# Lainshower/debiasing-multi-modal

Measured on AMD Instinct MI355X. Metric: images/sec (embed+adapter step), CLIP-RN50 224px bs=1024, higher is better.
Workload: dtype f32; 1 GPU; CLIP-RN50 224px encode_image + adapter(1024-128-1024) CE/SGD step, 1024 images/GPU, global batch 1024 (the metric's configuration, CLIP-RN50 224px bs=1024 on one GPU); global_batch=1024, batch_per_gpu=1024, parallelism=dp1, collective=none

## Files before the change

### debiasing-multi-modal_amd/_lib.py

```python
import ctypes
import glob
import os
import subprocess
from ctypes import c_double, c_float, c_int, c_int64, c_size_t, c_void_p

_HERE = os.path.dirname(os.path.abspath(__file__))
CSRC = os.path.join(_HERE, "csrc")
LIB_PATH = os.environ.get("DBMM_LIB") or os.path.join(_HERE, "libdbmm_hip.so")
INCLUDE = os.path.join(os.path.dirname(_HERE), "include")

_lib = None


def sources():
    return sorted(glob.glob(os.path.join(CSRC, "*.hip")))


KERNEL_SOURCES = (
    ("igemm_", ("igemm_f32.hip", "igemm_epilogue.inc", "common.h")),
    ("bottleneck_chain_kernel", ("bottleneck_chain.hip", "common.h")),
    ("bottleneck_chain8_kernel", ("bottleneck_chain8.hip", "common.h")),
    ("conv3x3_c32_kernel", ("conv_patch.hip", "common.h")),
    ("gemm_pair_8ph_kernel", ("gemm_pair_8ph.hip", "gemm_pair_8ph_epilogue.inc", "persistent_tiles.h", "common.h")),
    ("conv3x3_halo8", ("conv3x3_halo8.hip", "conv3x3_halo8_epilogue.inc", "persistent_tiles.h", "common.h")),
# ... 67 lines not shown

_SIGS = {
    "dbmm_set_option": [ctypes.c_char_p, _I],
    "dbmm_get_option": [ctypes.c_char_p, ctypes.POINTER(ctypes.c_int)],
    "dbmm_version": [],
    "dbmm_error_string": [_I],
    "dbmm_conv_bn_act": [_P, _P, _P, _P, _P, _L, _L, _L, _L, _L, _L, _L, _L, _L, _I, _P],
    "dbmm_conv1x1_bn_act": [_P, _P, _P, _P, _P, _L, _L, _L, _L, _L, _I, _P],
    "dbmm_conv3x3_bn_act": [_P, _P, _P, _P, _P, _L, _L, _L, _L, _L, _I, _P],
    "dbmm_gemm_bias_act": [_P, _L, _I, _P, _L, _I, _P, _P, _L, _P, _L, _L, _L, _L, _F, _I, _P],
    "dbmm_workspace_bytes_igemm": [],
    "dbmm_debug_last_igemm": [_P],
    "dbmm_conv_bn_act_ws": [_P, _P, _P, _P, _P, _L, _L, _L, _L, _L, _L, _L, _L, _L, _I, _I, _P, _Z, _P],
    "dbmm_gemm_bias_act_ws": [_P, _L, _I, _P, _L, _I, _P, _P, _L, _P, _L, _L, _L, _L, _F, _I, _P, _Z, _P],
    "dbmm_split_planes_bytes": [_L, _L],
    "dbmm_split_weight_planes": [_P, _P, _L, _L, _P],
    "dbmm_conv_bn_act_x3": [_P, _P, _P, _P, _P, _P, _L, _L, _L, _L, _L, _L, _L, _L, _L, _I, _I, _P, _Z, _P],
    "dbmm_split_planes_f16_bytes": [_L, _L],
    "dbmm_split_weight_planes_f16": [_P, _P, _L, _L, _I, _P],
    "dbmm_conv_bn_act_x2": [_P, _P, _P, _P, _I, _I, _P, _P, _P, _P, _P, _P, _L, _L, _L, _L, _L, _L, _L, _L, _L, _I, _I, _I, _P, _Z, _P],
    "dbmm_gemm_bias_act_x2": [_P, _L, _P, _P, _P, _I, _I, _L, _P, _P, _P, _L, _P, _L, _P, _L, _L, _L, _F, _I, _P, _Z, _P],
    "dbmm_gemm_dual_bn_act_x2": [_P, _L, _P, _P, _I, _L, _L, _P, _P, _L, _P, _P, _L, _L, _P, _P, _P, _L, _P, _L, _L, _I, _P, _Z, _P],
    "dbmm_bottleneck_chain_x2": [_P, _P, _P, _I, _P, _P, _P, _P, _P, _P, _P, _I, _P, _P, _P, _P, _L, _L, _L, _L, _L, _L, _P],
    "dbmm_bottleneck_chain_dual_x2": [_P, _P, _P, _I, _P, _P, _P, _P, _P, _P, _P, _P, _P, _I, _P, _P, _P, _P, _L, _L, _L, _L, _L, _P],
    "dbmm_gemm_f16": [_P, _L, _P, _L, _P, _P, _L, _P, _L, _L, _L, _L, _I, _P],
    "dbmm_gemm_f16_ws": [_P, _L, _P, _L, _P, _P, _L, _P, _L, _L, _L, _L, _I, _P, _Z, _P],
    "dbmm_mha_core_f16": [_P, _P, _L, _L, _L, _L, _I, _P],
    "dbmm_layernorm_f16": [_P, _L, _P, _P, _P, _L, _L, _L, _F, _P],
    "dbmm_conv1x1_bn_act_f16": [_P, _P, _P, _P, _P, _P, _L, _L, _L, _I, _P],
    "dbmm_conv1x1_bn_act_f16_ws": [_P, _P, _P, _P, _P, _P, _L, _L, _L, _I, _P, _Z, _P],
    "dbmm_conv1x1_dual_bn_act_f16": [_P, _P, _P, _P, _P, _P, _P, _P, _L, _L, _L, _L, _I, _P],
    "dbmm_bottleneck_chain_f16": [_P, _P, _P, _P, _P, _P, _P, _P, _P, _P, _L, _L, _L, _L, _P],
    "dbmm_bottleneck_chain_pool_f16": [_P, _P, _P, _P, _P, _P, _P, _P, _P, _P, _P, _L, _L, _L, _L, _L, _L, _P],
    "dbmm_bottleneck_chain_dual_f16": [_P, _P, _P, _P, _P, _P, _P, _P, _P, _P, _P, _P, _L, _L, _L, _L, _L, _P],
    "dbmm_conv3x3_bn_relu_f16": [_P, _P, _P, _P, _P, _L, _L, _L, _L, _L, _I, _P],
    "dbmm_conv_stem_s2_f16": [_P, _I, _P, _P, _P, _L, _L, _L, _L, _P],
    "dbmm_conv1x1_res_pool_f16": [_P, _P, _P, _P, _P, _P, _P, _L, _L, _L, _L, _L, _P],
    "dbmm_conv_stem_s2_bn_f16": [_P, _I, _P, _P, _P, _P, _L, _L, _L, _L, _P],
    "dbmm_avgpool2_f16": [_P, _P, _L, _L, _L, _L, _P],
    "dbmm_im2col_patch_f16": [_P, _I, _P, _L, _L, _L, _L, _P],
    "dbmm_vit_tokens_f16": [_P, _P, _P, _P, _L, _L, _L, _P],
    "dbmm_embed_gather_f16": [_P, _P, _P, _P, _L, _L, _L, _L, _P],
    "dbmm_gather_eot_f16": [_P, _P, _P, _L, _L, _L, _P],
    "dbmm_cast_f32_f16": [_P, _P, _L, _P],
    "dbmm_conv3x3_c32_bn_relu_x2": [_P, _P, _P, _I, _P, _P, _P, _P, _L, _L, _L, _L, _L, _I, _P],
    "dbmm_bottleneck_block_chain_x2": [_P, _P, _P, _I, _P, _P, _P, _I, _P, _P, _P, _P, _P, _P, _P, _P, _P, _P, _I, _P, _P, _P, _P,
                                       _L, _L, _L, _L, _L, _L, _P],
    "dbmm_gemm_bias_act_x3": [_P, _L, _P, _P, _L, _P, _P, _L, _P, _L, _L, _L, _L, _F, _I, _P, _Z, _P],
    "dbmm_gemm_batched": [_P, _L, _L, _I, _P, _L, _L, _I, _P, _L, _P, _L, _L, _L, _L, _L, _L, _F, _I, _P],
    "dbmm_gemm_pair_8ph": [_P, _L, _P, _P, _I, _L, _P, _P, _P, _L, _P, _L, _P, _L, _L, _L, _F, _I, _P],
    "dbmm_conv_stem_s2": [_P, _P, _P, _P, _P, _L, _L, _L, _L, _P],
    "dbmm_avgpool2d": [_P, _P, _L, _L, _L, _L, _L, _P],
    "dbmm_workspace_bytes_attnpool": [_L, _L, _L],
    "dbmm_attnpool": [_P, _P, _P, _P, _P, _P, _P, _P, _P, _L, _L, _L, _L, _L, _P, _Z, _P],
    "dbmm_attnpool_x": [_P, _I, _P, _P, _P, _P, _P, _P, _P, _P, _L, _L, _L, _L, _L, _P, _Z, _P],
    "dbmm_layernorm": [_P, _L, _P, _P, _P, _L, _L, _L, _F, _P, _P],
    "dbmm_mha_core": [_P, _P, _L, _L, _L, _L, _I, _P],
    "dbmm_mha_core_x2": [_P, _P, _P, _L, _L, _L, _L, _I, _P],
    "dbmm_embed_gather": [_P, _P, _P, _P, _L, _L, _L, _L, _P],
    "dbmm_im2col_patch": [_P, _P, _P, _L, _L, _L, _P],
    "dbmm_vit_tokens": [_P, _P, _P, _P, _L, _L, _L, _P],
    "dbmm_gather_eot": [_P, _P, _P, _L, _L, _L, _P],
    "dbmm_bn1d_stats": [_P, _L, _L, _F, _F, _P, _P, _P, _P, _P, _P],
    "dbmm_bn1d_relu": [_P, _P, _P, _P, _P, _P, _L, _L, _I, _F, _P],
    "dbmm_adapter_fwd": [_P] * 15 + [_L, _L, _L, _I, _F, _F, _P],
    "dbmm_workspace_bytes_adapter_bwd": [_L, _L, _L],
    "dbmm_adapter_bwd": [_P] * 15 + [_L, _L, _L, _P, _Z, _P],
    "dbmm_text_colnorm": [_P, _P, _L, _L, _P],
    "dbmm_l2norm_rows": [_P, _P, _L, _L, _P],
    "dbmm_colsum": [_P, _P, _L, _L, _P],
    "dbmm_l2norm_sim_ce_fwd": [_P, _P, _F, _P, _P, _F, _P, _P, _P, _P, _P, _L, _L, _L, _P],
    "dbmm_l2norm_sim_ce_bwd": [_P, _P, _F, _I, _P, _P, _P, _P, _F, _F, _P, _L, _L, _L, _P],
    "dbmm_sgd_momentum": [_L, _P, _P, _P, _P, _F, _F, _F, _I, _P],
    "dbmm_workspace_bytes_adapter_train_step": [_L, _L, _L, _I],
    "dbmm_adapter_train_step": [_P] * 26 + [_F, _P, _F, _F, _F, _F, _I, _P, _P, _P, _L, _L, _L, _L, _P, _Z, _P],
    "dbmm_group_dro_weights": [_P, _P, _P, _P, _P, _P, _L, _L, _F, _P],
    "dbmm_l2norm_sim_ce_bwd_weighted": [_P, _P, _F, _I, _P, _P, _P, _P, _P, _L, _F, _P, _L, _L, _L, _P],
    "dbmm_adapter_train_step_gdro": [_P] * 26 + [_F, _P, _F, _F, _F, _F, _I, _P, _P, _P, _P, _P, _F, _L, _L, _L, _L, _L, _P, _Z, _P],
    "dbmm_adapter_sweep_step_gdro": [_P, _L, _P, _L, _L, _P, _P, _P, _P, _P, _F, _P, _F, _P, _F, _F, _I, _P, _P, _P, _P, _P, _L, _I, _P, _F, _L, _L,
                                     _L, _L, _L, _P, _Z, _P],
    "dbmm_supcon_workspace_bytes": [_L, _L],
    "dbmm_supcon_fwd": [_P, _P, _F, _P, _F, _P, _P, _P, _P, _P, _L, _L, _P, _Z, _P],
    "dbmm_supcon_bwd": [_P, _P, _F, _P, _P, _F, _P, _F, _P, _L, _L, _P, _Z, _P],
    "dbmm_adapter_train_step_supcon": [_P] * 26 + [_F, _P, _F, _F, _F, _F, _I, _P, _P, _P, _F, _F, _P, _L, _L, _L, _L, _P, _Z, _P],
    "dbmm_supcon_sets_workspace_bytes": [_L, _L, _L],
    "dbmm_supcon_sets_fwd": [_P, _F, _F, _P, _P, _L, _L, _L, _L, _L, _P, _Z, _P],
    "dbmm_supcon_sets_bwd": [_P, _F, _F, _P, _L, _L, _L, _L, _L, _P, _Z, _P],
    "dbmm_workspace_bytes_adapter_train_step_sets": [_L, _L, _L, _L],
    "dbmm_adapter_train_step_sets": [_P] * 16 + [_F, _F, _F, _I, _F, _F, _P, _P, _L, _L, _L, _L, _L, _L, _P, _Z, _P],
    "dbmm_workspace_bytes_adapter_sweep_step": [_L, _L, _L, _L, _I],
    "dbmm_adapter_sweep_step": [_P, _L, _P, _L, _L, _P, _P, _P, _P, _P, _F, _P, _F, _P, _F, _F, _I, _P, _P, _P, _P, _P, _L, _I, _L, _L, _L, _L, _L,
                                _P, _Z, _P],
    "dbmm_workspace_bytes_adapter_sweep_eval": [_L, _L, _L, _L, _I],
    "dbmm_adapter_sweep_eval": [_P, _L, _P, _L, _P, _P, _P, _P, _F, _P, _F, _P, _P, _P, _P, _L, _L, _L, _L, _L, _L, _P, _Z, _P],
    "dbmm_workspace_bytes_linear_train_step": [_L, _L, _L],
    "dbmm_linear_train_step": [_P] * 6 + [_F, _F, _F, _I, _P, _P, _P, _L, _L, _L, _P, _Z, _P],
    "dbmm_workspace_bytes_linear_ce_fwd": [_L],
    "dbmm_linear_ce_fwd": [_P] * 7 + [_L, _L, _L, _P, _Z, _P],
    "dbmm_workspace_bytes_linear_sweep_step": [_L, _L, _L, _L],
    "dbmm_linear_sweep_step": [_P, _L, _P, _L, _L, _P, _P, _P, _P, _P, _P, _P, _F, _F, _I, _P, _P, _P, _P, _P, _L, _I, _L, _L, _L, _L, _P, _Z, _P],
    "dbmm_workspace_bytes_linear_sweep_eval": [_L, _L],
    "dbmm_linear_sweep_eval": [_P, _L, _P, _L, _P, _P, _P, _P, _P, _P, _P, _P, _L, _L, _L, _L, _L, _P, _Z, _P],
    "dbmm_weighted_mean": [_P, _P, _P, _L, _P],
    "dbmm_l2norm_sim_ce_bwd_rows": [_P, _P, _F, _I, _P, _P, _P, _P, _F, _F, _P, _L, _L, _L, _P],
    "dbmm_adapter_train_step_weighted": [_P] * 26 + [_F, _P, _F, _F, _F, _F, _I, _P, _P, _P, _P, _L, _L, _L, _L, _P, _Z, _P],
    "dbmm_adapter_sweep_step_weighted": [_P, _L, _P, _L, _L, _P, _P, _P, _P, _P, _F, _P, _F, _P, _F, _F, _I, _P, _P, _P, _P, _P, _L, _I, _P, _L,
# ... 99 lines not shown
```

### debiasing-multi-modal_amd/csrc/common.h

```cpp
#pragma once
#include <hip/hip_runtime.h>
#include <stdint.h>
#include <type_traits>
#include "../../include/dbmm.h"

typedef float f32x4 __attribute__((ext_vector_type(4)));
typedef float f32x16 __attribute__((ext_vector_type(16)));
typedef _Float16 f16x8 __attribute__((ext_vector_type(8)));
typedef _Float16 f16x4 __attribute__((ext_vector_type(4)));
typedef _Float16 f16x2 __attribute__((ext_vector_type(2)));
typedef unsigned short u16;
typedef unsigned int u32x2 __attribute__((ext_vector_type(2)));
typedef unsigned int u32x4 __attribute__((ext_vector_type(4)));

constexpr int DBMM_N_CU = 256;

#define DBMM_CHECK_LAUNCH()                      \
    do {                                         \
        hipError_t e__ = hipGetLastError();      \
        if (e__ != hipSuccess) return (int)e__;  \
    } while (0)

enum DbmmOpt {
    OPT_IGEMM_EPI_DIRECT, OPT_IGEMM_FAST, OPT_IGEMM_STREAMK, OPT_IGEMM_X3, OPT_IGEMM_X2, OPT_IGEMM_X2_BK, OPT_IGEMM_BK,
    OPT_IGEMM_HALO, OPT_IGEMM_HALO_POOL, OPT_IGEMM_BN256, OPT_IGEMM_BN256_KXK, OPT_GEMM_8PH, OPT_F16_8PH, OPT_F16_BN256,
    OPT_STEM_MFMA, OPT_MHA_VALU, OPT_CONV_PATCH, OPT_MHA_X2, OPT_ADAPTER_STEP_FUSED, OPT_CONV1X1_STREAM, OPT_CONV1X1_8PH, OPT_CHAIN8, OPT_CONV1X1_BN256, OPT_TAIL_SPLIT, OPT_HALO8, OPT_DUAL_8PH, OPT_MHA_SHORT, OPT_F16_CONV_8PH, OPT_CONV1X1_RES_STREAM, OPT_LINEAR_STEP_ONE_LAUNCH_MAX_B, DBMM_OPT_COUNT
};
int dbmm_opt(int id);

int dbmm_conv3x3_halo8(const float* x, const float* x_absmax, const void* w_plane_f16, int w_exp, const float* out_scale, const float* bias,
                       float* y, float* y_absmax, int64_t B, int64_t H, int64_t W, int64_t Cin, int64_t Cout, int act, int pool, int split,
                       void* workspace, size_t workspace_bytes, void* stream);

int dbmm_gemm_pair_8ph_ws(const float* a, int64_t lda, const float* a_absmax, const void* w_plane_f16, int w_exp, int64_t ldw,
                          const float* out_scale, const float* bias, const float* residual, int64_t ldr, float* c, int64_t ldc,
                          float* c_absmax, int64_t M, int64_t N, int64_t K, float alpha, int act, void* workspace, size_t workspace_bytes, void* stream);
int dbmm_gemm_dual_pair_8ph(const float* a, int64_t lda, const float* a_absmax, const void* w_plane_f16, int w_exp, int64_t ldw, int64_t K,
                            const float* out_scale, const float* a2, int64_t lda2, const float* a2_absmax, const void* w2_plane_f16, int64_t ldw2,
                            int64_t K2, const float* ratio, const float* bias, float* c, int64_t ldc, float* c_absmax, int64_t M, int64_t N, int act,
                            void* stream);

static inline int dbmm_cut_slices(int rem, int trips) {
    if (rem <= 0 || rem > DBMM_N_CU / 2) return 0;
    int S = DBMM_N_CU / rem;
    S = S < trips ? S : trips;
    S = S < 16 ? S : 16;
    return S >= 2 ? S : 0;
}

int dbmm_conv1x1_res_stream(const float* a, const float* a_absmax, const void* w_plane_f16, int w_exp, const float* scale, const float* bias,
                            const float* residual, float* y, float* y_pooled, float* y_absmax, int64_t M, int64_t Ho, int64_t Wo, int64_t K,
                            int64_t N, void* stream);

int dbmm_conv1x1_res_stream_f16(const void* x, const void* w, const float* scale, const float* bias, const void* residual, void* y, void* y_pooled,
                                int64_t M, int64_t Ho, int64_t Wo, int64_t Cin, int64_t Cout, void* stream);

float* dbmm_supcon_spare(void* workspace, int64_t B);

static inline bool dbmm_aligned16(const void* p) { return (((uintptr_t)p) & 15u) == 0; }

__device__ __forceinline__ float wave_sum(float v) {
#pragma unroll
    for (int o = 32; o > 0; o >>= 1) v += __shfl_xor(v, o, 64);
    return v;
}
__device__ __forceinline__ float wave_max(float v) {
#pragma unroll
    for (int o = 32; o > 0; o >>= 1) v = fmaxf(v, __shfl_xor(v, o, 64));
    return v;
}

__device__ __forceinline__ int xcd_first(int xcd, int n) {
    const int tq = n >> 3, trm = n & 7;
    return xcd < trm ? xcd * (tq + 1) : trm * (tq + 1) + (xcd - trm) * tq;
}
__device__ __forceinline__ int xcd_remap(int bid, int nwg) { return xcd_first(bid & 7, nwg) + (bid >> 3); }

constexpr unsigned OOR = 0x80000000u;
constexpr long long EXT_LIM = 0x7FFFFFF0LL;
// ... 36 lines not shown
```

### debiasing-multi-modal_amd/csrc/options.hip

```cpp
#include <atomic>
#include <ctype.h>
#include <stdlib.h>
#include <string.h>
#include "common.h"

namespace {

struct OptDef { const char* name; int def; };
const OptDef kOpts[DBMM_OPT_COUNT] = {
    {"igemm_epi_direct", 1},
    {"igemm_fast", 1},
    {"igemm_streamk", 1},
    {"igemm_x3", 1},
    {"igemm_x2", 1},
    {"igemm_x2_bk", 32},
    {"igemm_bk", 0},
    {"igemm_halo", 1},
    {"igemm_halo_pool", 2},
    {"igemm_bn256", 1},
    {"igemm_bn256_kxk", 1},
    {"gemm_8ph", 1},
    {"f16_8ph", 1},
    {"f16_bn256", 1},
    {"stem_mfma", 1},
    {"mha_valu", 0},
    {"conv_patch", 1},
    {"mha_x2", 1},
    {"adapter_step_fused", 1},
    {"conv1x1_stream", 1},
    {"conv1x1_8ph", 1},
    {"chain8", 0},
    {"conv1x1_bn256", 0},
    {"tail_split", 1},
    {"halo8", 1},
    {"dual_8ph", 1},
    {"mha_short", 1},
    {"f16_conv_8ph", 1},
    {"conv1x1_res_stream", 1},
    {"linear_step_one_launch_max_b", 512},
};

std::atomic<int> g_val[DBMM_OPT_COUNT];

struct Seed {
    Seed() {
        for (int i = 0; i < DBMM_OPT_COUNT; ++i) {
            char env[64] = "DBMM_";
            size_t n = strlen(env);
            for (const char* c = kOpts[i].name; *c && n + 1 < sizeof(env); ++c) env[n++] = (char)toupper((unsigned char)*c);
            env[n] = 0;
            const char* e = getenv(env);
            g_val[i].store(e ? atoi(e) : kOpts[i].def, std::memory_order_relaxed);
        }
    }
} g_seed;

int find(const char* name) {
    if (!name) return -1;
    for (int i = 0; i < DBMM_OPT_COUNT; ++i)
        if (!strcmp(name, kOpts[i].name)) return i;
    return -1;
}

}

int dbmm_opt(int id) { return g_val[id].load(std::memory_order_relaxed); }

extern "C" int dbmm_set_option(const char* name, int value) {
    const int i = find(name);
    if (i < 0) return DBMM_E_ARG;
    g_val[i].store(value, std::memory_order_relaxed);
    return DBMM_OK;
}

extern "C" int dbmm_get_option(const char* name, int* value) {
    const int i = find(name);
    if (i < 0 || !value) return DBMM_E_ARG;
    *value = g_val[i].load(std::memory_order_relaxed);
    return DBMM_OK;
}
```

### debiasing-multi-modal_amd/csrc/resnet_ops.hip

```cpp
#include <stdlib.h>
#include "common.h"

namespace {

template <int COUT>
__global__ __launch_bounds__(256) void stem_s2_kernel(const float* __restrict__ x, const float* __restrict__ w,
                                                      const float* __restrict__ bias, float* __restrict__ y,
                                                      float* __restrict__ y_absmax, int B, int H, int W, int Ho,
                                                      int Wo) {
    constexpr int Cout = COUT, PITCH = COUT + 4;
    __shared__ __attribute__((aligned(16))) float sw[28 * COUT];
    __shared__ __attribute__((aligned(16))) float stage[256 * PITCH];
    for (int i = threadIdx.x; i < 27 * Cout; i += blockDim.x) sw[i] = w[i];
    for (int i = threadIdx.x; i < Cout; i += blockDim.x) sw[27 * Cout + i] = bias ? bias[i] : 0.f;
    __syncthreads();
    const long long m0 = (long long)blockIdx.x * blockDim.x, m = m0 + threadIdx.x;
    const long long M = (long long)B * Ho * Wo;
    float omax = 0.f;
    if (m < M) {
    const int wo = (int)(m % Wo), ho = (int)((m / Wo) % Ho), n = (int)(m / ((long long)Wo * Ho));
    float xin[27];
#pragma unroll
    for (int kh = 0; kh < 3; ++kh)
#pragma unroll
// ... 267 lines not shown
         i += (long long)gridDim.x * blockDim.x) {
        const int c = (int)(i % C4);
        long long t = i / C4;
        const int wo = (int)(t % Wo); t /= Wo;
        const int ho = (int)(t % Ho);
        const long long n = t / Ho;
        const f32x4* src = (const f32x4*)x + ((n * H + (long long)ho * k) * W + (long long)wo * k) * C4 + c;
        f32x4 s = {0.f, 0.f, 0.f, 0.f};
        for (int a = 0; a < k; ++a)
            for (int b = 0; b < k; ++b) s += src[((long long)a * W + b) * C4];
        ((f32x4*)y)[i] = s * inv;
    }
}

template <int XH>
__global__ __launch_bounds__(256) void attnpool_tokens_kernel(const void* __restrict__ x,
                                                              const float* __restrict__ pos,
                                                              float* __restrict__ t, int HW, int C4, int Lp) {
    const int b = blockIdx.y;
    const int c = blockIdx.x * blockDim.x + threadIdx.x;
    if (c >= C4) return;
    const f32x4* pp = (const f32x4*)pos + c;
    f32x4* tb = (f32x4*)t + (long long)b * Lp * C4 + c;
    f32x4 s = {0.f, 0.f, 0.f, 0.f};
    for (int j = 0; j < HW; ++j) {
        f32x4 v;
        if constexpr (XH) {
            const f16x4 h = ((const f16x4*)x)[((long long)b * HW + j) * C4 + c];
            v = (f32x4){(float)h[0], (float)h[1], (float)h[2], (float)h[3]};
        } else {
            v = ((const f32x4*)x)[((long long)b * HW + j) * C4 + c];
        }
        s += v;
        tb[(long long)(j + 1) * C4] = v + pp[(long long)(j + 1) * C4];
    }
    tb[0] = s * (1.f / (float)HW) + pp[0];
    for (int j = HW + 1; j < Lp; ++j) tb[(long long)j * C4] = (f32x4){0.f, 0.f, 0.f, 0.f};
}

__global__ __launch_bounds__(256) void softmax_rows_kernel(float* __restrict__ s, int rows, int L, int Lp) {
    const int row = blockIdx.x * 4 + (threadIdx.x >> 6), lane = threadIdx.x & 63;
    if (row >= rows) return;
    float* r = s + (long long)row * Lp;
    float m = -INFINITY;
    for (int j = lane; j < L; j += 64) m = fmaxf(m, r[j]);
    m = wave_max(m);
    float sum = 0.f;
    for (int j = lane; j < L; j += 64) sum += expf(r[j] - m);
    sum = wave_sum(sum);
    const float inv = 1.f / sum;
    for (int j = lane; j < Lp; j += 64) r[j] = (j < L) ? expf(r[j] - m) * inv : 0.f;
}

}

extern "C" int dbmm_conv_stem_s2(const float* x_nchw, const float* w, const float* bias, float* y_nhwc,
                                 float* y_absmax, int64_t B, int64_t H, int64_t W, int64_t Cout, void* stream) {
    if (!x_nchw || !w || !y_nhwc) return DBMM_E_ARG;
    if (B <= 0 || H <= 0 || W <= 0 || Cout <= 0 || (Cout & 7) || Cout > 512) return DBMM_E_SHAPE;
    if (!dbmm_aligned16(y_nhwc)) return DBMM_E_ALIGN;
    const int64_t Ho = (H + 2 - 3) / 2 + 1, Wo = (W + 2 - 3) / 2 + 1;
    const int64_t M = B * Ho * Wo;
    if (M > INT32_MAX) return DBMM_E_SHAPE;
    const dim3 g((unsigned)((M + 255) / 256));
    hipStream_t s = (hipStream_t)stream;
#define DBMM_STEM(C) hipLaunchKernelGGL(stem_s2_kernel<C>, g, dim3(256), 0, s, x_nchw, w, bias, y_nhwc, y_absmax, (int)B, (int)H, (int)W, (int)Ho, (int)Wo)
    if (dbmm_opt(OPT_STEM_MFMA) && (Cout == 32 || Cout == 64) && 3 * H * W * 8 < 0x7FFFFFF0LL && (M + 31) / 32 <= INT32_MAX) {
        const int n_blocks = (int)((M + 31) / 32);
        const int wgs = (n_blocks + 3) / 4 < 256 * 8 ? (n_blocks + 3) / 4 : 256 * 8;
        if (Cout == 32)
            hipLaunchKernelGGL(stem_s2_mfma_kernel<1>, dim3(wgs), dim3(256), 0, s, x_nchw, w, bias, y_nhwc, y_absmax, (int)B, (int)H,
                               (int)W, (int)Ho, (int)Wo, n_blocks);
        else
            hipLaunchKernelGGL(stem_s2_mfma_kernel<2>, dim3(wgs), dim3(256), 0, s, x_nchw, w, bias, y_nhwc, y_absmax, (int)B, (int)H,
                               (int)W, (int)Ho, (int)Wo, n_blocks);
        DBMM_CHECK_LAUNCH();
        return DBMM_OK;
    }
    if (Cout == 32) DBMM_STEM(32);
    else if (Cout == 40) DBMM_STEM(40);
    else if (Cout == 48) DBMM_STEM(48);
    else if (Cout == 64) DBMM_STEM(64);
    else
        hipLaunchKernelGGL(stem_s2_generic_kernel, g, dim3(256), (size_t)(28 * Cout) * sizeof(float), s, x_nchw, w, bias, y_nhwc,
                           y_absmax, (int)B, (int)H, (int)W, (int)Ho, (int)Wo, (int)Cout);
#undef DBMM_STEM
    DBMM_CHECK_LAUNCH();
    return DBMM_OK;
}

extern "C" int dbmm_avgpool2d(const float* x, float* y, int64_t B, int64_t H, int64_t W, int64_t C, int64_t k,
                              void* stream) {
    if (!x || !y) return DBMM_E_ARG;
    if (B <= 0 || H <= 0 || W <= 0 || C <= 0 || k <= 0 || (C & 3) || H % k || W % k) return DBMM_E_SHAPE;
    if (!dbmm_aligned16(x) || !dbmm_aligned16(y)) return DBMM_E_ALIGN;
    const int64_t Ho = H / k, Wo = W / k, C4 = C / 4;
    const long long total = (long long)B * Ho * Wo * C4;
    const long long blocks = (total + 255) / 256;
    const unsigned grid = (unsigned)(blocks < 16384 ? blocks : 16384);
    hipLaunchKernelGGL(avgpool_kernel, dim3(grid), dim3(256), 0, (hipStream_t)stream, x, y, (int)H, (int)W,
                       (int)C4, (int)Ho, (int)Wo, (int)k, total);
    DBMM_CHECK_LAUNCH();
    return DBMM_OK;
}

extern "C" size_t dbmm_workspace_bytes_attnpool(int64_t B, int64_t HW, int64_t C) {
    const int64_t Lp = (HW + 1 + 3) / 4 * 4, heads = C / 64;
    return (size_t)(B * Lp * C + 2 * B * C + B * heads * C + B * heads * Lp) * sizeof(float);
}

extern "C" int dbmm_attnpool_x(const void* x, int x_is_f16, const float* pos, const float* wq, const float* bq,
                               const float* wkv, const float* bkv, const float* wc, const float* bc, float* out,
                               int64_t B, int64_t HW, int64_t C, int64_t heads, int64_t Dout, void* workspace,
                               size_t workspace_bytes, void* stream);

extern "C" int dbmm_attnpool(const float* x, const float* pos, const float* wq, const float* bq,
                             const float* wkv, const float* bkv, const float* wc, const float* bc, float* out,
                             int64_t B, int64_t HW, int64_t C, int64_t heads, int64_t Dout, void* workspace,
                             size_t workspace_bytes, void* stream) {
    return dbmm_attnpool_x(x, 0, pos, wq, bq, wkv, bkv, wc, bc, out, B, HW, C, heads, Dout, workspace, workspace_bytes, stream);
}

extern "C" int dbmm_attnpool_x(const void* x, int x_is_f16, const float* pos, const float* wq, const float* bq,
                               const float* wkv, const float* bkv, const float* wc, const float* bc, float* out,
                               int64_t B, int64_t HW, int64_t C, int64_t heads, int64_t Dout, void* workspace,
                               size_t workspace_bytes, void* stream) {
    if (!x || !pos || !wq || !wkv || !bkv || !wc || !out || !workspace) return DBMM_E_ARG;
    if (B <= 0 || HW <= 0 || C <= 0 || heads <= 0 || C != heads * 64 || (C & 3) || Dout <= 0 || B > 65535)
        return DBMM_E_SHAPE;
    if (workspace_bytes < dbmm_workspace_bytes_attnpool(B, HW, C)) return DBMM_E_WORKSPACE;
    if (!dbmm_aligned16(x) || !dbmm_aligned16(pos) || !dbmm_aligned16(workspace)) return DBMM_E_ALIGN;
    const int64_t L = HW + 1, Lp = (L + 3) / 4 * 4;
    float* tok = (float*)workspace;
    float* q = tok + B * Lp * C;
    float* U = q + B * C;
    float* S = U + B * heads * C;
    float* o = S + B * heads * Lp;
    hipStream_t s = (hipStream_t)stream;
    const int C4 = (int)(C / 4);
    if (x_is_f16)
        hipLaunchKernelGGL(attnpool_tokens_kernel<1>, dim3((C4 + 255) / 256, (unsigned)B), dim3(256), 0, s, x, pos, tok, (int)HW, C4, (int)Lp);
    else
        hipLaunchKernelGGL(attnpool_tokens_kernel<0>, dim3((C4 + 255) / 256, (unsigned)B), dim3(256), 0, s, x, pos, tok, (int)HW, C4, (int)Lp);
    DBMM_CHECK_LAUNCH();
    int rc;
    rc = dbmm_gemm_bias_act(tok, Lp * C, 0, wq, C, 0, bq, nullptr, 0, q, C, B, C, C, 0.125f, DBMM_ACT_NONE, stream);
    if (rc) return rc;
    rc = dbmm_gemm_batched(q, C, 64, 0, wkv, C, 64 * C, 1, nullptr, 0, U, heads * C, C, B, C, 64, heads, 1.f,
                           DBMM_ACT_NONE, stream);
    if (rc) return rc;
    rc = dbmm_gemm_batched(U, C, heads * C, 0, tok, C, Lp * C, 0, nullptr, 0, S, Lp, heads * Lp, heads, Lp, C, B, 1.f,
                           DBMM_ACT_NONE, stream);
    if (rc) return rc;
    const int64_t rows = B * heads;
    hipLaunchKernelGGL(softmax_rows_kernel, dim3((unsigned)((rows + 3) / 4)), dim3(256), 0, s, S, (int)rows, (int)L,
                       (int)Lp);
    DBMM_CHECK_LAUNCH();
    float* Sx = U;
    rc = dbmm_gemm_batched(S, Lp, heads * Lp, 0, tok, C, Lp * C, 1, nullptr, 0, Sx, C, heads * C, heads, C, Lp, B, 1.f,
                           DBMM_ACT_NONE, stream);
    if (rc) return rc;
    rc = dbmm_gemm_batched(Sx, heads * C, C, 0, wkv + C * C, C, 64 * C, 0, bkv + C, 64, o, C, 64, B, 64, C, heads, 1.f,
                           DBMM_ACT_NONE, stream);
    if (rc) return rc;
    return dbmm_gemm_bias_act(o, C, 0, wc, C, 0, bc, nullptr, 0, out, Dout, B, Dout, C, 1.f, DBMM_ACT_NONE, stream);
}
```

### debiasing-multi-modal_amd/ops.py

```python
import ctypes
import math
import os

import numpy as np
import torch

from . import _lib
from ._lib import check, ptr, require_cuda, stream

ACT_NONE, ACT_RELU, ACT_QUICKGELU = 0, 1, 2


class DbmmUnsupported(_lib.DbmmError):
    """a wrapper's C entry answered DBMM_E_UNSUPPORTED (no kernel for this valid request)"""


def set_option(name, value):
    old = get_option(name)
    check(_lib.lib().dbmm_set_option(name.encode(), int(value)), f"set_option({name})")
    return old


def get_option(name):
    v = ctypes.c_int()
# ... 379 lines not shown
    check(rc, "bottleneck_block_chain_x2")
    t.__exit__(None, None, None)
    return x, y1n


def bottleneck_chain_dual(y2, y2_absmax, c3, a2, a2_absmax, ds, ratio, bias, c1, x_absmax=None, y1_absmax=None):
    require_cuda(y2, a2)
    _f32c(y2); _f32c(a2)
    K, K2 = y2.shape[-1], a2.shape[-1]
    N, P = c3["ph"].shape[1], c1["ph"].shape[1]
    M = y2.numel() // K
    if (c3["ph"].shape[0] != 1 or ds["ph"].shape[0] != 1 or c1["ph"].shape[0] != 1 or a2.numel() // K2 != M
            or K != 64 or K2 != 64 or N % 64 or P not in (64, 128) or M % 4):
        return None
    x = _empty(tuple(y2.shape[:-1]) + (N,), device=y2.device, dtype=torch.float32)
    y1 = _empty(tuple(y2.shape[:-1]) + (P,), device=y2.device, dtype=torch.float32)
    global _chain_tag
    _chain_tag = f"bottleneck_chain_kernel<{K}, {P}, 0, 1>"
    t = _Timed(M, N, K + K2 + P, -1, 0, 4 * (M * K + M * K2 + M * N + M * P) + 2 * (N * K + N * K2 + P * N))
    t.__enter__()
    rc = _lib.lib().dbmm_bottleneck_chain_dual_x2(ptr(y2), ptr(y2_absmax), ptr(c3["ph"]), int(c3["we"]), ptr(c3["sc"]), ptr(bias),
                                                 ptr(a2), ptr(a2_absmax), ptr(ds["ph"]), ptr(ratio), ptr(x), ptr(x_absmax),
                                                 ptr(c1["ph"]), int(c1["we"]), ptr(c1["sc"]), ptr(c1["b"]), ptr(y1),
                                                 ptr(y1_absmax), M, K, K2, N, P, stream())
    if rc == _lib.E_UNSUPPORTED:
        return None
    check(rc, "bottleneck_chain_dual_x2")
    t.__exit__(None, None, None)
    return x, y1


def conv_stem_s2(x_nchw, w, bias, y_absmax=None):
    require_cuda(x_nchw, w)
    _f32c(x_nchw); _f32c(w)
    B, C, H, W = x_nchw.shape
    if C != 3:
        raise _lib.DbmmError("stem conv expects 3 input channels")
    Cout = w.shape[-1]
    y = _empty((B, (H - 1) // 2 + 1, (W - 1) // 2 + 1, Cout), device=x_nchw.device, dtype=torch.float32)
    check(_lib.lib().dbmm_conv_stem_s2(ptr(x_nchw), ptr(w), ptr(bias), ptr(y), ptr(y_absmax), B, H, W, Cout, stream()),
          "conv_stem_s2")
    return y


def avgpool2d(x, k):
    require_cuda(x)
    _f32c(x)
    B, H, W, C = x.shape
    y = _empty((B, H // k, W // k, C), device=x.device, dtype=torch.float32)
    check(_lib.lib().dbmm_avgpool2d(ptr(x), ptr(y), B, H, W, C, k, stream()), "avgpool2d")
    return y


def attnpool(x, pos, wq, bq, wkv, bkv, wc, bc, heads):
    require_cuda(x)
    if x.dtype != torch.float16:
        _f32c(x)
    elif not x.is_contiguous():
        raise _lib.DbmmError("attnpool: expected a contiguous tensor")
    B, H, W, C = x.shape
    HW = H * W
    Dout = wc.shape[0]
    if tuple(pos.shape) != (HW + 1, C):
        raise RuntimeError(f"attnpool: positional embedding {tuple(pos.shape)} does not match a {H} x {W} x {C} feature map "
                           f"(expected ({HW + 1}, {C})): the input resolution differs from the one the model was built for")
    if (tuple(wq.shape) != (C, C) or tuple(wkv.shape) != (2 * C, C) or wc.shape[1] != C or bq.numel() != C or bkv.numel() != 2 * C
            or bc.numel() != Dout):
        raise RuntimeError(f"attnpool: projection shapes {tuple(wq.shape)}, {tuple(wkv.shape)}, {tuple(wc.shape)} do not match C = {C}")
    for t in (pos, wq, bq, wkv, bkv, wc, bc):
        require_cuda(t)
        _f32c(t)
    nbytes = _lib.lib().dbmm_workspace_bytes_attnpool(B, HW, C)
    ws = _empty(nbytes // 4, device=x.device, dtype=torch.float32)
    out = _empty((B, Dout), device=x.device, dtype=torch.float32)
    check(_lib.lib().dbmm_attnpool_x(ptr(x), int(x.dtype == torch.float16), ptr(pos), ptr(wq), ptr(bq), ptr(wkv), ptr(bkv), ptr(wc), ptr(bc),
                                     ptr(out), B, HW, C, heads, Dout, ptr(ws), nbytes, stream()), "attnpool")
    return out


def layernorm(x, gamma, beta, rows=None, ldx=None, eps=1e-5, y_absmax=None):
    require_cuda(x)
    E = gamma.numel()
    if rows is None:
        rows = x.numel() // E
    if ldx is None:
        ldx = E
    _sized("layernorm beta", beta, E)
    if ldx < E or x.numel() < (rows - 1) * ldx + E:
        raise RuntimeError(f"layernorm: input {tuple(x.shape)} for {rows} rows of {E} at pitch {ldx}")
    y = _empty((rows, E), device=x.device, dtype=torch.float32)
    check(_lib.lib().dbmm_layernorm(ptr(x), ldx, ptr(gamma), ptr(beta), ptr(y), E, rows, E, eps, ptr(y_absmax), stream()),
          "layernorm")
    return y


def mha_core(qkv, B, L, E, heads, causal, qkv_absmax=None):
    require_cuda(qkv)
    if qkv.numel() != B * L * 3 * E or E != heads * 64:
        raise RuntimeError(f"mha_core: qkv {tuple(qkv.shape)} for B = {B}, L = {L}, E = {E}, {heads} heads of 64")
    out = _empty((B * L, E), device=qkv.device, dtype=torch.float32)
    if qkv_absmax is not None and get_option("mha_x2"):
        with _TimedTag("mha_pair_kernel", 4.0 * B * heads * L * L * 64, 4 * (B * L * 4 * E)):
            check(_lib.lib().dbmm_mha_core_x2(ptr(qkv), ptr(qkv_absmax), ptr(out), B, L, E, heads, int(causal), stream()),
                  "mha_core_x2")
        return out
    with _TimedTag("mha_mfma_kernel", 4.0 * B * heads * L * L * 64, 4 * (B * L * 4 * E)):
# ... 1301 lines not shown
```

### include/dbmm.h

```cpp
#ifndef DBMM_H
#define DBMM_H

#include <stddef.h>
#include <stdint.h>

#ifdef __cplusplus
extern "C" {
#endif

#define DBMM_OK 0
#define DBMM_E_SHAPE (-1)
#define DBMM_E_ALIGN (-2)
#define DBMM_E_WORKSPACE (-3)
#define DBMM_E_ARG (-4)
#define DBMM_E_UNSUPPORTED (-5)

#define DBMM_WL_TAP_MAJOR 0
#define DBMM_WL_CHUNK_MAJOR 1
#define DBMM_WL_CHUNK32_MAJOR 2

#define DBMM_ACT_NONE 0
#define DBMM_ACT_RELU 1
#define DBMM_ACT_QUICKGELU 2

// ... 110 lines not shown
                                   const float* bias, void* x_out, const void* w1, const float* scale1, const float* bias1, void* y1_out,
                                   int64_t M, int64_t K, int64_t K2, int64_t N, int64_t P, void* stream);
int dbmm_conv1x1_bn_act_f16_ws(const void* x, const void* w, const float* scale, const float* bias, const void* residual, void* y,
                               int64_t M, int64_t Cin, int64_t Cout, int act, void* workspace, size_t workspace_bytes,
                               void* stream);
int dbmm_conv1x1_res_pool_f16(const void* x, const void* w, const float* scale, const float* bias, const void* residual, void* y,
                              void* y_pooled, int64_t B, int64_t Ho, int64_t Wo, int64_t Cin, int64_t Cout, void* stream);
int dbmm_conv3x3_bn_relu_f16(const void* x, const void* w, const float* scale, const float* bias, void* y, int64_t B, int64_t H,
                             int64_t W, int64_t Cin, int64_t Cout, int pool, void* stream);
int dbmm_conv_stem_s2_f16(const void* x_nchw, int x_is_f16, const float* w, const float* bias, void* y_nhwc, int64_t B, int64_t H,
                          int64_t W, int64_t Cout, void* stream);
int dbmm_conv_stem_s2_bn_f16(const void* x_nchw, int x_is_f16, const float* w, const float* scale, const float* bias, void* y_nhwc,
                             int64_t B, int64_t H, int64_t W, int64_t Cout, void* stream);
int dbmm_avgpool2_f16(const void* x, void* y, int64_t B, int64_t H, int64_t W, int64_t C, void* stream);
int dbmm_mha_core_f16(const void* qkv, void* out, int64_t B, int64_t L, int64_t E, int64_t heads, int causal, void* stream);
int dbmm_layernorm_f16(const void* x, int64_t ldx, const float* gamma, const float* beta, void* y, int64_t ldy,
                       int64_t rows, int64_t E, float eps, void* stream);
int dbmm_im2col_patch_f16(const void* x_nchw, int x_is_f16, void* out, int64_t B, int64_t R, int64_t P, int64_t Kp,
                          void* stream);
int dbmm_vit_tokens_f16(const void* patches, const float* cls, const float* pos, void* out, int64_t B, int64_t L,
                        int64_t W, void* stream);
int dbmm_embed_gather_f16(const int32_t* tokens, const float* table, const float* pos, void* out, int64_t n, int64_t L,
                          int64_t W, int64_t vocab, void* stream);
int dbmm_gather_eot_f16(const int32_t* tokens, const void* x, void* out, int64_t n, int64_t L, int64_t W, void* stream);
int dbmm_cast_f32_f16(const float* x, void* y, int64_t n, void* stream);

size_t dbmm_workspace_bytes_preprocess(int64_t nrows, int64_t R);
int dbmm_resize_crop_normalize_u8(const uint8_t* img_hwc, int64_t H, int64_t W, const int32_t* h_bounds,
                                  const int32_t* h_coeffs, int64_t h_ksize, const int32_t* v_bounds,
                                  const int32_t* v_coeffs, int64_t v_ksize, int64_t row0, int64_t nrows,
                                  int64_t R, const float* mean3, const float* std3, float* out_chw,
                                  uint8_t* out_u8_hwc, void* workspace, size_t workspace_bytes, void* stream);
int dbmm_resize_crop_normalize_u8_batch(const uint8_t* img_bhwc, int64_t B, int64_t H, int64_t W, const int32_t* h_bounds,
                                  const int32_t* h_coeffs, int64_t h_ksize, const int32_t* v_bounds,
                                  const int32_t* v_coeffs, int64_t v_ksize, int64_t row0, int64_t nrows,
                                  int64_t R, const float* mean3, const float* std3, float* out_chw,
                                  uint8_t* out_u8_hwc, void* workspace, size_t workspace_bytes, void* stream);

void dbmm_debug_last_igemm(int* out11);

int dbmm_gemm_batched(const float* a, int64_t lda, int64_t stride_a, int trans_a, const float* w,
                      int64_t ldw, int64_t stride_w, int trans_w, const float* bias,
                      int64_t stride_bias, float* c, int64_t ldc, int64_t stride_c, int64_t M,
                      int64_t N, int64_t K, int64_t batch, float alpha, int act, void* stream);


int dbmm_conv_stem_s2(const float* x_nchw, const float* w, const float* bias, float* y_nhwc,
                      float* y_absmax, int64_t B, int64_t H, int64_t W, int64_t Cout, void* stream);

int dbmm_avgpool2d(const float* x, float* y, int64_t B, int64_t H, int64_t W, int64_t C,
                   int64_t k, void* stream);

size_t dbmm_workspace_bytes_attnpool(int64_t B, int64_t HW, int64_t C);
int dbmm_attnpool(const float* x, const float* pos, const float* wq, const float* bq,
                  const float* wkv, const float* bkv, const float* wc, const float* bc,
                  float* out, int64_t B, int64_t HW, int64_t C, int64_t heads, int64_t Dout,
                  void* workspace, size_t workspace_bytes, void* stream);
int dbmm_attnpool_x(const void* x, int x_is_f16, const float* pos, const float* wq, const float* bq,
                    const float* wkv, const float* bkv, const float* wc, const float* bc, float* out,
                    int64_t B, int64_t HW, int64_t C, int64_t heads, int64_t Dout, void* workspace,
                    size_t workspace_bytes, void* stream);


int dbmm_layernorm(const float* x, int64_t ldx, const float* gamma, const float* beta, float* y,
                   int64_t ldy, int64_t rows, int64_t E, float eps, float* y_absmax, void* stream);

int dbmm_mha_core(const float* qkv, float* out, int64_t B, int64_t L, int64_t E, int64_t heads,
                  int causal, void* stream);

int dbmm_mha_core_x2(const float* qkv, const float* qkv_absmax, float* out, int64_t B, int64_t L, int64_t E,
                     int64_t heads, int causal, void* stream);

int dbmm_embed_gather(const int32_t* tokens, const float* table, const float* pos, float* out,
                      int64_t n, int64_t L, int64_t W, int64_t vocab, void* stream);

int dbmm_im2col_patch(const float* x_nchw, float* out, float* out_absmax, int64_t B, int64_t R, int64_t P, void* stream);

int dbmm_vit_tokens(const float* patches, const float* cls, const float* pos, float* out,
                    int64_t B, int64_t L, int64_t W, void* stream);

int dbmm_gather_eot(const int32_t* tokens, const float* x, float* out, int64_t n, int64_t L,
                    int64_t W, void* stream);


int dbmm_bn1d_stats(const float* h, int64_t B, int64_t H, float eps, float momentum, float* mean,
                    float* invstd, float* running_mean, float* running_var, int64_t* nbt,
                    void* stream);

int dbmm_bn1d_relu(const float* h, const float* mean, const float* invstd, const float* gamma,
                   const float* beta, float* r, int64_t B, int64_t H, int var_mode, float eps,
                   void* stream);

int dbmm_adapter_fwd(const float* x, const float* w1, const float* b1, const float* gamma,
                     const float* beta, float* running_mean, float* running_var, int64_t* nbt,
                     const float* w2, const float* b2, float* h, float* mean, float* invstd,
                     float* r, float* z, int64_t B, int64_t D, int64_t H, int train, float eps,
                     float momentum, void* stream);

size_t dbmm_workspace_bytes_adapter_bwd(int64_t B, int64_t D, int64_t H);
int dbmm_adapter_bwd(const float* x, const float* dz, const float* h, const float* mean,
                     const float* invstd, const float* r, const float* gamma, const float* beta,
                     const float* w2, float* dw1, float* db1, float* dgamma, float* dbeta,
                     float* dw2, float* db2, int64_t B, int64_t D, int64_t H, void* workspace,
                     size_t workspace_bytes, void* stream);

int dbmm_l2norm_rows(const float* x, float* y, int64_t B, int64_t D, void* stream);
// ... 208 lines not shown
```

Measured before the change: 36560 images/sec.

## Fuse attention-pool token build, scores, softmax and value mix into one core kernel

Adds a fused attention-pool path for short token counts. A small kernel computes only the mean token plus its positional embedding; the per-head score GEMM, softmax and probability-weighted token sum run in a single MFMA core kernel that rebuilds tokens from x+pos on the fly, so the large token tensor is never written. This removes a full B×L×C token materialisation and the separate score/softmax/mix launches, and shrinks the workspace. The cost is a complex hand-written kernel with per-L template instances and LDS reductions, which could be slower than the tuned GEMM path.

New measurement: 36730 images/sec, median of 6. No clear change (+0.5%).

```diff
diff --git a/debiasing-multi-modal_amd/_lib.py b/debiasing-multi-modal_amd/_lib.py
--- a/debiasing-multi-modal_amd/_lib.py
+++ b/debiasing-multi-modal_amd/_lib.py
@@ -143,6 +143,7 @@
     "dbmm_conv_stem_s2": [_P, _P, _P, _P, _P, _L, _L, _L, _L, _P],
     "dbmm_avgpool2d": [_P, _P, _L, _L, _L, _L, _L, _P],
     "dbmm_workspace_bytes_attnpool": [_L, _L, _L],
+    "dbmm_attnpool_plan": [_L, _L, _L, _L],
     "dbmm_attnpool": [_P, _P, _P, _P, _P, _P, _P, _P, _P, _L, _L, _L, _L, _L, _P, _Z, _P],
     "dbmm_attnpool_x": [_P, _I, _P, _P, _P, _P, _P, _P, _P, _P, _L, _L, _L, _L, _L, _P, _Z, _P],
     "dbmm_layernorm": [_P, _L, _P, _P, _P, _L, _L, _L, _F, _P, _P],
diff --git a/debiasing-multi-modal_amd/csrc/common.h b/debiasing-multi-modal_amd/csrc/common.h
--- a/debiasing-multi-modal_amd/csrc/common.h
+++ b/debiasing-multi-modal_amd/csrc/common.h
@@ -24,7 +24,7 @@
 enum DbmmOpt {
     OPT_IGEMM_EPI_DIRECT, OPT_IGEMM_FAST, OPT_IGEMM_STREAMK, OPT_IGEMM_X3, OPT_IGEMM_X2, OPT_IGEMM_X2_BK, OPT_IGEMM_BK,
     OPT_IGEMM_HALO, OPT_IGEMM_HALO_POOL, OPT_IGEMM_BN256, OPT_IGEMM_BN256_KXK, OPT_GEMM_8PH, OPT_F16_8PH, OPT_F16_BN256,
-    OPT_STEM_MFMA, OPT_MHA_VALU, OPT_CONV_PATCH, OPT_MHA_X2, OPT_ADAPTER_STEP_FUSED, OPT_CONV1X1_STREAM, OPT_CONV1X1_8PH, OPT_CHAIN8, OPT_CONV1X1_BN256, OPT_TAIL_SPLIT, OPT_HALO8, OPT_DUAL_8PH, OPT_MHA_SHORT, OPT_F16_CONV_8PH, OPT_CONV1X1_RES_STREAM, OPT_LINEAR_STEP_ONE_LAUNCH_MAX_B, DBMM_OPT_COUNT
+    OPT_STEM_MFMA, OPT_MHA_VALU, OPT_CONV_PATCH, OPT_MHA_X2, OPT_ADAPTER_STEP_FUSED, OPT_CONV1X1_STREAM, OPT_CONV1X1_8PH, OPT_CHAIN8, OPT_CONV1X1_BN256, OPT_TAIL_SPLIT, OPT_HALO8, OPT_DUAL_8PH, OPT_MHA_SHORT, OPT_F16_CONV_8PH, OPT_CONV1X1_RES_STREAM, OPT_LINEAR_STEP_ONE_LAUNCH_MAX_B, OPT_ATTNPOOL_FUSED, DBMM_OPT_COUNT
 };
 int dbmm_opt(int id);
 
diff --git a/debiasing-multi-modal_amd/csrc/options.hip b/debiasing-multi-modal_amd/csrc/options.hip
--- a/debiasing-multi-modal_amd/csrc/options.hip
+++ b/debiasing-multi-modal_amd/csrc/options.hip
@@ -38,6 +38,7 @@
     {"f16_conv_8ph", 1},
     {"conv1x1_res_stream", 1},
     {"linear_step_one_launch_max_b", 512},
+    {"attnpool_fused", 1},
 };
 
 std::atomic<int> g_val[DBMM_OPT_COUNT];
diff --git a/debiasing-multi-modal_amd/csrc/resnet_ops.hip b/debiasing-multi-modal_amd/csrc/resnet_ops.hip
--- a/debiasing-multi-modal_amd/csrc/resnet_ops.hip
+++ b/debiasing-multi-modal_amd/csrc/resnet_ops.hip
@@ -343,6 +343,186 @@
     for (int j = lane; j < Lp; j += 64) r[j] = (j < L) ? expf(r[j] - m) * inv : 0.f;
 }
 
+template <int XH>
+__device__ __forceinline__ f32x4 ap_f32x4(std::conditional_t<XH != 0, f16x4, f32x4> v) {
+    if constexpr (XH) return (f32x4){(float)v[0], (float)v[1], (float)v[2], (float)v[3]};
+    else return v;
+}
+
+template <int XH>
+__global__ __launch_bounds__(256) void attnpool_mean_kernel(const void* __restrict__ x, const float* __restrict__ pos,
+                                                            float* __restrict__ t0, int HW, int C4) {
+    using XV = std::conditional_t<XH != 0, f16x4, f32x4>;
+    const int b = blockIdx.y;
+    const int c = blockIdx.x * blockDim.x + threadIdx.x;
+    if (c >= C4) return;
+    const XV* xb = (const XV*)x + (long long)b * HW * C4 + c;
+    f32x4 s = {0.f, 0.f, 0.f, 0.f};
+#pragma unroll 8
+    for (int j = 0; j < HW; ++j) s += ap_f32x4<XH>(xb[(long long)j * C4]);
+    ((f32x4*)t0)[(long long)b * C4 + c] = s * (1.f / (float)HW) + ((const f32x4*)pos)[c];
+}
+
+__device__ __forceinline__ f32x4 ap_ld(__amdgpu_buffer_rsrc_t r, unsigned voff, unsigned soff, f32x4) {
+    return __builtin_bit_cast(f32x4, __builtin_amdgcn_raw_buffer_load_b128(r, voff, soff, 0));
+}
+__device__ __forceinline__ f16x4 ap_ld(__amdgpu_buffer_rsrc_t r, unsigned voff, unsigned soff, f16x4) {
+    return __builtin_bit_cast(f16x4, __builtin_amdgcn_raw_buffer_load_b64(r, voff, soff, 0));
+}
+__device__ __forceinline__ float ap_ld(__amdgpu_buffer_rsrc_t r, unsigned voff, unsigned soff, float) {
+    return __builtin_bit_cast(float, __builtin_amdgcn_raw_buffer_load_b32(r, voff, soff, 0));
+}
+__device__ __forceinline__ _Float16 ap_ld(__amdgpu_buffer_rsrc_t r, unsigned voff, unsigned soff, _Float16) {
+    return __builtin_bit_cast(_Float16, __builtin_amdgcn_raw_buffer_load_b16(r, voff, soff, 0));
+}
+
+constexpr int AP_MAX_L = 160;
+constexpr int ap_kc(int nb) { return nb <= 2 ? 128 : 64; }
+constexpr int ap_minw(int nb) { return nb <= 2 ? 4 : 1; }
+
+template <int XH, int NB, int KC>
+__global__ __launch_bounds__(KC * 4, ap_minw(NB)) void attnpool_core_kernel(const void* __restrict__ x, const float* __restrict__ pos,
+                                                                            const float* __restrict__ t0, float* u, int HW, int C,
+                                                                            int heads) {
+    using XV = std::conditional_t<XH != 0, f16x4, f32x4>;
+    using XS = std::conditional_t<XH != 0, _Float16, float>;
+    constexpr int NW = KC / 16;
+    constexpr int LD = KC + 4;
+    constexpr int SLD = NB * 32 + 4;
+    constexpr unsigned XB = sizeof(XS);
+    __shared__ __attribute__((aligned(16))) float lds[(NB + 1) * 32 * LD];
+    float* Ul = lds;
+    float* Tl = lds + 32 * LD;
+    float* Sl = lds;
+    const int tid = threadIdx.x, lane = tid & 63, wave = tid >> 6;
+    const int fr = lane & 31, fh = lane >> 5;
+    const int b = blockIdx.x, h0 = blockIdx.y * 32;
+    const int L = HW + 1;
+    const int hn = heads - h0 < 32 ? heads - h0 : 32;
+    const __amdgpu_buffer_rsrc_t rx = desc(x, (long long)(b + 1) * HW * C * XB, (long long)b * HW * C * XB);
+    const __amdgpu_buffer_rsrc_t rp = desc(pos, (long long)L * C * 4, 0);
+    const __amdgpu_buffer_rsrc_t rt = desc(t0, (long long)(b + 1) * C * 4, (long long)b * C * 4);
+    const __amdgpu_buffer_rsrc_t ru = desc(u, ((long long)b * heads + h0 + hn) * C * 4, ((long long)b * heads + h0) * C * 4);
+
+    const int c4 = tid % (KC / 4), r16 = tid / (KC / 4);
+    const unsigned e0 = (unsigned)r16 * C + c4 * 4;
+    f32x4 ur[2], pr[2 * NB], t0r;
+    XV xr[2 * NB];
+    auto fetch = [&](int kc) {
+        const unsigned k0 = kc * KC;
+        const bool in = k0 + c4 * 4 < (unsigned)C;
+#pragma unroll
+        for (int i = 0; i < 2; ++i) ur[i] = ap_ld(ru, in && i * 16 + r16 < hn ? e0 * 4 : OOR, ((unsigned)(i * 16) * C + k0) * 4, f32x4{});
+        t0r = ap_ld(rt, in && r16 == 0 ? c4 * 16 : OOR, k0 * 4, f32x4{});
+#pragma unroll
+        for (int p = 0; p < 2 * NB; ++p) {
+            const int tok = p * 16 + r16;
+            const bool ok = in && tok >= 1 && tok < L;
+            xr[p] = ap_ld(rx, ok ? (p ? e0 : e0 - C) * XB : OOR, ((unsigned)(p ? p * 16 - 1 : 0) * C + k0) * XB, XV{});
+            pr[p] = ap_ld(rp, ok ? e0 * 4 : OOR, ((unsigned)(p * 16) * C + k0) * 4, f32x4{});
+        }
+    };
+    auto stash = [&]() {
+#pragma unroll
+        for (int i = 0; i < 2; ++i) *(f32x4*)(Ul + (i * 16 + r16) * LD + c4 * 4) = ur[i];
+#pragma unroll
+        for (int p = 0; p < 2 * NB; ++p) {
+            f32x4 v = ap_f32x4<XH>(xr[p]) + pr[p];
+            if (p == 0 && r16 == 0) v = t0r;
+            *(f32x4*)(Tl + (p * 16 + r16) * LD + c4 * 4) = v;
+        }
+    };
+    f32x16 acc[NB], tot[NB];
+#pragma unroll
+    for (int n = 0; n < NB; ++n) { acc[n] = (f32x16)(0.f); tot[n] = (f32x16)(0.f); }
+    const int nchunk = (C + KC - 1) / KC;
+    fetch(0);
+    for (int kc = 0; kc < nchunk; ++kc) {
+        __syncthreads();
+        stash();
+        __syncthreads();
+        if (kc + 1 < nchunk) fetch(kc + 1);
+        if (kc && (kc & 7) == 0) {
+#pragma unroll
+            for (int n = 0; n < NB; ++n) { tot[n] += acc[n]; acc[n] = (f32x16)(0.f); }
+        }
+#pragma unroll
+        for (int g = 0; g < 2; ++g) {
+            const int ch = wave * 16 + g * 8 + fh * 4;
+            const f32x4 af = *(const f32x4*)(Ul + fr * LD + ch);
+#pragma unroll
+            for (int n = 0; n < NB; ++n) {
+                const f32x4 wf = *(const f32x4*)(Tl + (n * 32 + fr) * LD + ch);
+#pragma unroll
+                for (int s = 0; s < 4; ++s) acc[n] = __builtin_amdgcn_mfma_f32_32x32x2f32(af[s], wf[s], acc[n], 0, 0, 0);
+            }
+        }
+    }
+#pragma unroll
+    for (int n = 0; n < NB; ++n) acc[n] += tot[n];
+    for (int w = 0; w < NW; ++w) {
+        __syncthreads();
+        if (wave == w) {
+#pragma unroll
+            for (int n = 0; n < NB; ++n)
+#pragma unroll
+                for (int r = 0; r < 16; ++r) {
+                    float* d = Sl + ((r & 3) + 8 * (r >> 2) + 4 * fh) * SLD + n * 32 + fr;
+                    *d = w ? *d + acc[n][r] : acc[n][r];
+                }
+        }
+    }
+    __syncthreads();
+
+    for (int i = 0; i < 32 / NW; ++i) {
+        float* r = Sl + (wave * (32 / NW) + i) * SLD;
+        float m = -INFINITY;
+        for (int j = lane; j < L; j += 64) m = fmaxf(m, r[j]);
+        m = wave_max(m);
+        float sum = 0.f;
+        for (int j = lane; j < L; j += 64) sum += expf(r[j] - m);
+        sum = wave_sum(sum);
+        const float inv = 1.f / sum;
+        for (int j = lane; j < NB * 32; j += 64) r[j] = (j < L) ? expf(r[j] - m) * inv : 0.f;
+    }
+    __syncthreads();
+
+    constexpr int NQ = NB * 16;
+    float* zb = u + ((long long)b * heads + h0) * C;
+    const int nq = (L + 1) >> 1;
+    for (int cb = wave; cb < (C >> 5); cb += NW) {
+        const unsigned c = cb * 32 + fr, c2 = c + (unsigned)fh * C;
+        const float t0v = ap_ld(rt, c * 4, 0, float{});
+        XS xv[NQ];
+        float pv[NQ];
+#pragma unroll
+        for (int q = 0; q < NQ; ++q)
+            if (q < nq) {
+                const bool both = 2 * q + 1 < L;
+                xv[q] = ap_ld(rx, (q && both ? c2 : c) * XB, (unsigned)(q ? 2 * q - 1 : 0) * C * XB, XS{});
+                pv[q] = ap_ld(rp, (both ? c2 : c) * 4, (unsigned)(2 * q) * C * 4, float{});
+            }
+        f32x16 z = (f32x16)(0.f);
+#pragma unroll
+        for (int g = 0; g < NQ / 4; ++g)
+            if (g * 4 < nq) {
+                const f32x4 pa = *(const f32x4*)(Sl + fr * SLD + g * 8), pb = *(const f32x4*)(Sl + fr * SLD + g * 8 + 4);
+                const float pf[4] = {fh ? pa[1] : pa[0], fh ? pa[3] : pa[2], fh ? pb[1] : pb[0], fh ? pb[3] : pb[2]};
+#pragma unroll
+                for (int s = 0; s < 4; ++s) {
+                    const int q = g * 4 + s, tok = 2 * q + fh;
+                    const float tv = (q >= nq || tok >= L) ? 0.f : (tok == 0 ? t0v : (float)xv[q] + pv[q]);
+                    z = __builtin_amdgcn_mfma_f32_32x32x2f32(pf[s], tv, z, 0, 0, 0);
+                }
+            }
+#pragma unroll
+        for (int r = 0; r < 16; ++r) {
+            const int hr = (r & 3) + 8 * (r >> 2) + 4 * fh;
+            if (hr < hn) zb[(unsigned)hr * C + c] = z[r];
+        }
+    }
+}
+
 }
 
 extern "C" int dbmm_conv_stem_s2(const float* x_nchw, const float* w, const float* bias, float* y_nhwc,
@@ -395,9 +575,16 @@
     return DBMM_OK;
 }
 
+extern "C" int dbmm_attnpool_plan(int64_t B, int64_t HW, int64_t C, int64_t heads) {
+    (void)B; (void)C; (void)heads;
+    if (!dbmm_opt(OPT_ATTNPOOL_FUSED)) return 0;
+    return HW + 1 <= AP_MAX_L ? 1 : 2;
+}
+
 extern "C" size_t dbmm_workspace_bytes_attnpool(int64_t B, int64_t HW, int64_t C) {
     const int64_t Lp = (HW + 1 + 3) / 4 * 4, heads = C / 64;
-    return (size_t)(B * Lp * C + 2 * B * C + B * heads * C + B * heads * Lp) * sizeof(float);
+    const int64_t tok = dbmm_attnpool_plan(B, HW, C, heads) == 1 ? 0 : B * Lp * C;
+    return (size_t)(tok + 2 * B * C + B * heads * C + B * heads * Lp) * sizeof(float);
 }
 
 extern "C" int dbmm_attnpool_x(const void* x, int x_is_f16, const float* pos, const float* wq, const float* bq,
@@ -422,19 +609,51 @@
     if (workspace_bytes < dbmm_workspace_bytes_attnpool(B, HW, C)) return DBMM_E_WORKSPACE;
     if (!dbmm_aligned16(x) || !dbmm_aligned16(pos) || !dbmm_aligned16(workspace)) return DBMM_E_ALIGN;
     const int64_t L = HW + 1, Lp = (L + 3) / 4 * 4;
+    hipStream_t s = (hipStream_t)stream;
+    const int C4 = (int)(C / 4);
+    int rc;
+    if (dbmm_attnpool_plan(B, HW, C, heads) == 1) {
+        float* q = (float*)workspace;
+        float* U = q + B * C;
+        float* o = U + B * heads * C + B * heads * Lp;
+        float* t0 = o;
+        const dim3 gm((C4 + 255) / 256, (unsigned)B);
+        if (x_is_f16) hipLaunchKernelGGL(attnpool_mean_kernel<1>, gm, dim3(256), 0, s, x, pos, t0, (int)HW, C4);
+        else hipLaunchKernelGGL(attnpool_mean_kernel<0>, gm, dim3(256), 0, s, x, pos, t0, (int)HW, C4);
+        DBMM_CHECK_LAUNCH();
+        rc = dbmm_gemm_bias_act(t0, C, 0, wq, C, 0, bq, nullptr, 0, q, C, B, C, C, 0.125f, DBMM_ACT_NONE, stream);
+        if (rc) return rc;
+        rc = dbmm_gemm_batched(q, C, 64, 0, wkv, C, 64 * C, 1, nullptr, 0, U, heads * C, C, B, C, 64, heads, 1.f,
+                               DBMM_ACT_NONE, stream);
+        if (rc) return rc;
+        const dim3 gc((unsigned)B, (unsigned)((heads + 31) / 32));
+#define DBMM_AP_CORE(XH, NB) hipLaunchKernelGGL((attnpool_core_kernel<XH, NB, ap_kc(NB)>), gc, dim3(ap_kc(NB) * 4), 0, s, x, pos, t0, U, (int)HW, (int)C, (int)heads)
+#define DBMM_AP_CORE_NB(NB) do { if (x_is_f16) DBMM_AP_CORE(1, NB); else DBMM_AP_CORE(0, NB); } while (0)
+        switch ((L + 31) / 32) {
+            case 1: DBMM_AP_CORE_NB(1); break;
+            case 2: DBMM_AP_CORE_NB(2); break;
+            case 3: DBMM_AP_CORE_NB(3); break;
+            case 4: DBMM_AP_CORE_NB(4); break;
+            default: DBMM_AP_CORE_NB(5); break;
+        }
+#undef DBMM_AP_CORE_NB
+#undef DBMM_AP_CORE
+        DBMM_CHECK_LAUNCH();
+        rc = dbmm_gemm_batched(U, heads * C, C, 0, wkv + C * C, C, 64 * C, 0, bkv + C, 64, o, C, 64, B, 64, C, heads, 1.f,
+                               DBMM_ACT_NONE, stream);
+        if (rc) return rc;
+        return dbmm_gemm_bias_act(o, C, 0, wc, C, 0, bc, nullptr, 0, out, Dout, B, Dout, C, 1.f, DBMM_ACT_NONE, stream);
+    }
     float* tok = (float*)workspace;
     float* q = tok + B * Lp * C;
     float* U = q + B * C;
     float* S = U + B * heads * C;
     float* o = S + B * heads * Lp;
-    hipStream_t s = (hipStream_t)stream;
-    const int C4 = (int)(C / 4);
     if (x_is_f16)
         hipLaunchKernelGGL(attnpool_tokens_kernel<1>, dim3((C4 + 255) / 256, (unsigned)B), dim3(256), 0, s, x, pos, tok, (int)HW, C4, (int)Lp);
     else
         hipLaunchKernelGGL(attnpool_tokens_kernel<0>, dim3((C4 + 255) / 256, (unsigned)B), dim3(256), 0, s, x, pos, tok, (int)HW, C4, (int)Lp);
     DBMM_CHECK_LAUNCH();
-    int rc;
     rc = dbmm_gemm_bias_act(tok, Lp * C, 0, wq, C, 0, bq, nullptr, 0, q, C, B, C, C, 0.125f, DBMM_ACT_NONE, stream);
     if (rc) return rc;
     rc = dbmm_gemm_batched(q, C, 64, 0, wkv, C, 64 * C, 1, nullptr, 0, U, heads * C, C, B, C, 64, heads, 1.f,
diff --git a/debiasing-multi-modal_amd/ops.py b/debiasing-multi-modal_amd/ops.py
--- a/debiasing-multi-modal_amd/ops.py
+++ b/debiasing-multi-modal_amd/ops.py
@@ -455,6 +455,10 @@
     return y
 
 
+def attnpool_plan(B, HW, C, heads):
+    return _lib.lib().dbmm_attnpool_plan(B, HW, C, heads)
+
+
 def attnpool(x, pos, wq, bq, wkv, bkv, wc, bc, heads):
     require_cuda(x)
     if x.dtype != torch.float16:
diff --git a/include/dbmm.h b/include/dbmm.h
--- a/include/dbmm.h
+++ b/include/dbmm.h
@@ -186,6 +186,7 @@
                    int64_t k, void* stream);
 
 size_t dbmm_workspace_bytes_attnpool(int64_t B, int64_t HW, int64_t C);
+int dbmm_attnpool_plan(int64_t B, int64_t HW, int64_t C, int64_t heads);
 int dbmm_attnpool(const float* x, const float* pos, const float* wq, const float* bq,
                   const float* wkv, const float* bkv, const float* wc, const float* bc,
                   float* out, int64_t B, int64_t HW, int64_t C, int64_t heads, int64_t Dout,
```
